# moble/scri

Hardware: AMD Instinct MI355X
Metric: timesteps/sec for full BMS transform, l_max=16, 1e5 steps; fp64 (higher is better)
Workload: dtype f64

## Files before the change

scri_amd/csrc/engine_abd.hip:

```cpp
#include "engine.h"

static int transform_abd_impl(bms_ctx* c, const double* u, const void* raw, int mem, int64_t n_times, int ell_max,
                              const bms_transformation* tr, const bms_shard* sh, double* u_out, void* raw_out, int64_t* n_times_out,
                              int64_t* first_index_out);

extern "C" int bms_transform_abd_shard(bms_ctx* c, const double* u, const void* raw, int mem, int64_t n_times, int ell_max,
                                       const bms_transformation* tr, const bms_shard* sh, double* u_out, void* raw_out,
                                       int64_t* n_times_out, int64_t* first_index_out) try {
  if (!c) return BMS_ERR_INVALID;
  return with_smaller_chunks(c, [&] { return transform_abd_impl(c, u, raw, mem, n_times, ell_max, tr, sh, u_out, raw_out, n_times_out, first_index_out); });
} BMS_CATCH(c)

static int transform_abd_impl(bms_ctx* c, const double* u, const void* raw, int mem, int64_t n_times, int ell_max,
                              const bms_transformation* tr, const bms_shard* sh, double* u_out, void* raw_out, int64_t* n_times_out,
                              int64_t* first_index_out) {
  if (!u || !raw || !tr || !u_out || !raw_out || !n_times_out) return fail(c, BMS_ERR_INVALID, "NULL argument");
  if (!valid_mem(mem)) return fail(c, BMS_ERR_INVALID, "mem is BMS_HOST or BMS_DEVICE, got %d", mem);
  HIP_TRY(c, hipSetDevice(c->device));
  const int64_t n = n_times;
  int64_t t_lo, t_hi;
  time_window(n, sh, t_lo, t_hi);
  bool regular_mesh = true;
  int rc;
  begin_setup_reuse(c);
  KnotTables kt;
  if ((rc = knot_tables_ahead(c, u, n, sh, t_lo, t_hi, kt))) return rc;
  if (kt.axis_known) {
    rc = validate_transformation(c, n, u, tr, 2);
    regular_mesh = c->tcache.regular;
  } else
    rc = validate_common(c, n, u, tr, t_lo, t_hi, &regular_mesh, 2);
  if (rc) return rc;
  const bool short_series = n < 4;
  if (short_series && sh && !(sh->data_row0 == 0 && sh->data_rows == n && sh->col_parts <= 1))
    return fail(c, BMS_ERR_UNSUPPORTED, "a series of %lld samples cannot be sharded", (long long)n);
  if ((rc = refuse_sharded_graded_axis(c, regular_mesh, sh, n))) return rc;
  if (ell_max < 0 || tr->ell_max_out < 0) return fail(c, BMS_ERR_INVALID, "bad ell_max");
  if (ell_max > MAX_ELL) return fail(c, BMS_ERR_UNSUPPORTED, "ell_max = %d is beyond %d", ell_max, MAX_ELL);
  static const int spins[6] = {2, 1, 0, -1, -2, 2};
  const int nm = (ell_max + 1) * (ell_max + 1);
  const int n_out = (tr->ell_max_out + 1) * (tr->ell_max_out + 1);
  const int lst = tr->ell_max_supertranslation;
  const cplx* st = (const cplx*)tr->supertranslation;

  hipStream_t S = c->stream;
  std::vector<cplx> c1((size_t)(lst + 1) * (lst + 1)), c2((size_t)(lst + 1) * (lst + 1));
  for (int l = 0; l <= lst; ++l)
    for (int m = -l; m <= l; ++m) {
      const cplx a = st[LM_index(l, m, 0)];
      const double f1 = std::sqrt((double)l * (l + 1.0)) / std::sqrt(2.0);
      const double f2 = 0.5 * (std::sqrt((double)l * (l + 1.0)) * (l >= 1 ? std::sqrt((l - 1.0) * (l + 2.0)) : 0.0));
      c1[LM_index(l, m, 0)] = {f1 * a.re, f1 * a.im};
      c2[LM_index(l, m, 0)] = {f2 * a.re, f2 * a.im};
    }
  const double* v = tr->boost_velocity;
  const cplx cv[4] = {{0, 0},
                      {v[0] * std::sqrt(2 * M_PI / 3), v[1] * std::sqrt(2 * M_PI / 3)},
                      {v[2] * std::sqrt(4 * M_PI / 3), 0},
                      {-v[0] * std::sqrt(2 * M_PI / 3), v[1] * std::sqrt(2 * M_PI / 3)}};
  SynthesisPlan syn5[5];
  const bool no_boost = v[0] == 0 && v[1] == 0 && v[2] == 0;
  std::vector<double> ring_theta;
  bool sep = !(sh && sh->col_parts > 1) && tr->n_theta >= 3 && !c->opt.on(OPT_NO_SEPARABLE_SYNTHESIS) &&
             (no_boost || (axis_boost_pays(c, (ell_max + 1) * (ell_max + 1), tr->n_theta, tr->n_phi) &&
                           large_synthesis_route(c, tr->n_theta, tr->n_phi, 0, ell_max) && separable_rotor_grid(c, tr, ring_theta)));
  for (int si = 0; si < 5 && sep; ++si) {
    if ((rc = build_synthesis(c, tr->n_theta, tr->n_phi, si - 2, 0, ell_max, syn5[si], no_boost ? nullptr : &ring_theta))) return rc;
    sep = syn5[si].large;
  }
  PixelTables T;
  DevPixel DP;
  PieceTables* shared = c->async_pieces ? static_cast<PieceTables*>(c->piece_tables) : nullptr;
  if (shared && c->piece_tables_valid) {
    T = shared->T;
    DP = shared->DP;
  } else {
    if ((rc = device_pixel_tables(c, tr, T, 2, 0, 0, &c1, &c2, cv, DP, sep ? 0 : column_plan(c, tr, n_out), nullptr, nullptr, nullptr, reuse_tag(sh)))) return rc;
    if (shared) {
      shared->T = T;
      shared->DP = DP;
      c->piece_tables_valid = true;
    }
  }
  const int n_cols = T.n_pix;
  const bool col_split = sh && sh->col_parts > 1;
  int cA, cB;
  if ((rc = column_range(c, sh, n_cols, cA, cB))) return rc;
  const int n_pix = cB - cA;
  int64_t i_lo, i_hi;
  if (!cached_window(c, true, i_lo, i_hi)) {
    output_window_abd(T, u, n, i_lo, i_hi);
    keep_window(c, true, i_lo, i_hi);
  }
  int64_t row0 = 0, rows_avail = n, fs_out = n;
  if (sh) {
    row0 = sh->data_row0;
    rows_avail = sh->data_rows;
    if (row0 < 0 || rows_avail < 0 || row0 + rows_avail > n || sh->out_i1 < sh->out_i0) return fail(c, BMS_ERR_INVALID, "bad shard description");
    i_lo = std::max(i_lo, sh->out_i0);
    i_hi = std::max(i_lo, std::min(i_hi, sh->out_i1));
    fs_out = sh->out_i1 - sh->out_i0;
  }
  const int64_t n_new = i_hi - i_lo;
  *n_times_out = n_new;
  if (first_index_out) *first_index_out = i_lo;
  for (int64_t i = 0; i < n_new; ++i) u_out[i] = (u[i_lo + i] - T.tt) / T.gamma;
  if (n_new == 0) return BMS_OK;
  double *d_rot = DP.rotors, *d_skewa = DP.skew_a + cA, *d_skewb = DP.skew_b + cA, *d_alpha = DP.alpha + cA, *d_ethk = DP.ethk + 2 * cA,
         *d_etha = DP.etha + 2 * cA, *d_ethetha = DP.ethetha + 2 * cA, *d_ik = DP.ik + cA, *d_ik3 = DP.ik3 + cA;
  const bool bsg = n >= 8 && regular_mesh && !c->opt.on(OPT_NO_BSPLINE);
  if (short_series) {
    void* vp;
    if ((rc = upload(c, "times", u, 8 * (size_t)n, &vp))) return rc;
    kt.d_x = (double*)vp;
  } else if ((rc = knot_tables_of_call(c, u, n, t_lo, t_hi, row0, rows_avail, bsg, shared, kt)))
    return rc;

  const long long P2 = 2LL * n_pix, ldg = round_up(P2, 16), ldb = round_up(2LL * n_cols, 128);
  const int K = 2 * nm;
  const long long brows = round_up(K, 16);
  double *d_B[5], *d_At[5] = {nullptr, nullptr, nullptr, nullptr, nullptr};
  long long ld_at = 0;
  AnalysisPlan ana[5];
  const bool sigma_eval = !sep && bsg && !short_series && rows_avail >= 8 && !c->opt.on(OPT_NO_ABD_SIGMA_EVAL);
  PixelCache& pc = c->pcache;
  const bool keep_B = !sep && pc.in_use && sizeof(double) * (size_t)brows * ldb <= SETUP_CACHE_MAX_BYTES;
  const bool have_B = keep_B && pc.B5_valid && pc.B5_ell_max == ell_max && pc.B5_cols == n_cols && pc.B5_sigma == sigma_eval;
  if (keep_B && !have_B) pc.B5_valid = false;
  for (int si = 0; si < 5; ++si) {
    char nm1[32], tag[16];
    snprintf(nm1, sizeof nm1, keep_B ? "pc_abd_B%d" : "abd_B%d", si);
    snprintf(tag, sizeof tag, "abd%d", si);
    if (!sep && have_B) {
      d_B[si] = pc.d_B5[si];
    } else if (!sep) {
      if ((rc = dev_buf_t(c, nm1, (size_t)brows * ldb, &d_B[si]))) return rc;
      HIP_TRY(c, hipMemsetAsync(d_B[si], 0, sizeof(double) * brows * ldb, S));
      TIMED(c, BMS_TAG_SETUP, launch_swsh_matrix_complex(S, d_rot, n_cols, si - 2, 0, ell_max, d_B[si], ldb));
    }
    if ((rc = build_analysis(c, tag, T.n_theta, T.n_phi, si - 2, 0, tr->ell_max_out, ana[si]))) return rc;
    if (col_split && n_pix > 0) {
      snprintf(nm1, sizeof nm1, "abd_At%d", si);
      if ((rc = part_analysis_matrix(c, ana[si], nm1, n_cols, DP.col_of_pixel, &d_At[si], &ld_at))) return rc;
    }
  }

  const long long ldG = (!col_split && analysis_reads_contiguous_rows(ana[2])) ? P2 : ldg;
  const double* d_raw;
  if ((rc = stage_in(c, "in_data", raw, mem, (size_t)6 * rows_avail * nm * 16, &d_raw))) return rc;
  double* d_out = (double*)raw_out;
  if (mem == BMS_HOST)
    if ((rc = dev_buf_t(c, "out_data", (size_t)6 * fs_out * n_out * 2, &d_out))) return rc;
  const bool fused_mix = sep && no_boost && bsg && !short_series && !c->opt.on(OPT_NO_FUSED_ABD_MIX) && large_synthesis_route(c, tr->n_theta, tr->n_phi, 0, ell_max) &&
                         abd_mix6_supported(tr->n_theta, tr->n_phi, ell_max);
  const long long ld_af = round_up(2LL * (nm + 1), 16);
  double* d_Af = nullptr;
  if (fused_mix) {
    if ((rc = dev_buf_t(c, "abd_Af", (size_t)6 * rows_avail * ld_af, &d_Af))) return rc;
    for (int f = 0; f < 6; ++f)
      TIMED(c, BMS_TAG_SPLINE_FORWARD, launch_bspline_forward_modes(S, d_raw + (size_t)f * rows_avail * nm * 2, 2LL * nm, nm, d_Af + (size_t)f * rows_avail * ld_af,
                                                                    ld_af, row0, rows_avail, n, kt.d_bsfwd, SPLINE_TILE, SPLINE_HALO, 1));
    if ((rc = rotate_into_grid_frame(c, tr, d_Af, 6 * rows_avail, ld_af / 2, 0, ell_max))) return rc;
  } else if (sep) {
    if ((rc = rotated_input_in_grid_frame(c, tr, "abd_rot_in", mem, &d_raw, 6 * rows_avail, nm, 0, ell_max))) return rc;
  }

  if (n_pix == 0) {
    for (int f = 0; f < 6; ++f) {
      if (mem == BMS_HOST)
        std::memset((char*)raw_out + (size_t)f * fs_out * n_out * 16, 0, (size_t)n_new * n_out * 16);
      else
        HIP_TRY(c, hipMemsetAsync(d_out + (size_t)f * fs_out * n_out * 2, 0, (size_t)n_new * n_out * 16, S));
    }
    HIP_TRY(c, hipStreamSynchronize(S));
    return BMS_OK;
  }

  double* d_As = nullptr;
  if (sigma_eval) {
    if ((rc = dev_buf_t(c, "abd_As", (size_t)rows_avail * ld_af, &d_As))) return rc;
    TIMED(c, BMS_TAG_SPLINE_FORWARD, launch_bspline_solve_modes(S, d_raw + (size_t)5 * rows_avail * nm * 2, 2LL * nm, nm, d_As, ld_af, row0, rows_avail,
                                                                kt.d_bsfwd, kt.d_bstab, 1));
    if (brows < (long long)nm + 1 + 8) return fail(c, BMS_ERR_HIP, "internal: the spin-2 matrix has %lld rows, sigma's offset row needs %d", brows, nm + 9);
    if (!have_B) TIMED(c, BMS_TAG_SETUP, launch_negated_row(S, DP.ethetha, d_B[4] + (size_t)nm * ldb, 2 * n_cols));
  }
  if (keep_B && !have_B) {
    pc.B5_valid = true, pc.B5_sigma = sigma_eval, pc.B5_ell_max = ell_max, pc.B5_cols = n_cols;
    for (int si = 0; si < 5; ++si) pc.d_B5[si] = d_B[si];
  }

  BsplineSpread spread = skew_spread(T, cA, cB, u);
  spread.launches = c->bwd_launches;
  const double bytes_per_row = 19.0 * ldg * 8.0;
  ChunkPlan plan;
  if ((rc = plan_chunks(c, c->ws_limit, bytes_per_row, n_new, regular_mesh, n, "six ", n_cols, plan))) return rc;
  for (int64_t c0 = i_lo; c0 < i_hi; c0 += plan.chunk) {
    const int64_t c1_ = std::min<int64_t>(c0 + plan.chunk, i_hi);
    int64_t g0, g1;
    if ((rc = chunk_rows(c, T, u, n, regular_mesh, c0, c1_, row0, rows_avail, g0, g1))) return rc;
    const int64_t rows_in = g1 - g0, rows_out = c1_ - c0;
    double *d_Y = nullptr, *d_R, *d_G;
    if (!fused_mix)
      if ((rc = dev_buf_t(c, "Y", (size_t)6 * rows_in * ldg, &d_Y))) return rc;
    if ((rc = dev_buf_t(c, "R", (size_t)6 * rows_in * ldg, &d_R))) return rc;
    if ((rc = dev_buf_t(c, "G", (size_t)6 * rows_out * ldG, &d_G))) return rc;
    AbdGrids grids;
    if (fused_mix) {
      const size_t f_stride = (size_t)rows_in * (2 * ell_max + 1) * large_analysis_jp(T.n_theta) * 2;
      double* d_F6;
      if ((rc = dev_buf_t(c, "Fsyn6", 6 * f_stride, &d_F6))) return rc;
      const double* F6[6];
      double* out6[6];
      for (int f = 0; f < 6; ++f) {
        F6[f] = d_F6 + f * f_stride;
        out6[f] = d_R + (size_t)f * rows_in * ldg;
        TIMED(c, BMS_TAG_GEMM_SYNTHESIS, launch_theta_synthesis(S, d_Af + ((size_t)f * rows_avail + (g0 - row0)) * ld_af, ld_af, rows_in, T.n_theta, 0, ell_max,
                                                                syn5[spins[f] + 2].d_T, d_F6 + f * f_stride));
      }
      TIMED(c, BMS_TAG_GEMM_SYNTHESIS, launch_phi_synthesis_mix6(S, F6, rows_in, T.n_theta, T.n_phi, ell_max, d_etha, d_ethetha,
                                                                 d_Af + (size_t)(g0 - row0) * ld_af + 2LL * nm, ld_af, out6, ldg));
    }
    for (int f = 0; f < 6 && !fused_mix; ++f) {
      grids.y[f] = d_Y + (size_t)f * rows_in * ldg;
      if (f == 5 && sigma_eval) continue;
      if (sep) {
        if ((rc = run_synthesis(c, syn5[spins[f] + 2], d_raw + ((size_t)f * rows_avail + (g0 - row0)) * nm * 2, 2LL * nm, rows_in, nullptr, grids.y[f], ldg)))
          return rc;
      } else
      {
        const int skip = spins[f] * spins[f] < nm ? spins[f] * spins[f] : 0;
        TIMED(c, BMS_TAG_GEMM_SYNTHESIS,
              launch_zgemm3m(S, d_raw + ((size_t)f * rows_avail + (g0 - row0)) * nm * 2 + 2 * skip, 2LL * nm, d_B[spins[f] + 2] + 2 * cA + (size_t)skip * ldb, ldb,
                             grids.y[f], ldg, rows_in, n_pix, K / 2 - skip, nullptr, nullptr));
      }
    }
    if (fused_mix) {
    } else if (bsg) {
      AbdGrids elim;
      for (int f = 0; f < 6; ++f) elim.y[f] = d_R + (size_t)f * rows_in * ldg;
      TIMED(c, BMS_TAG_SPLINE_FORWARD, launch_abd_mix_forward(S, grids, elim, ldg, n_pix, g0, rows_in, kt.d_bsfwd, SPLINE_TILE, SPLINE_HALO, d_alpha, d_ethk,
                                                              d_etha, d_ethetha, d_ik, d_ik3, sigma_eval ? 5 : 6));
    } else {
      TIMED(c, BMS_TAG_POINTWISE,
            launch_abd_mix(S, grids, ldg, n_pix, rows_in, kt.d_x + g0, d_alpha, d_ethk, d_etha, d_ethetha, d_ik, d_ik3));
    }
    for (int f = 0; f < 6; ++f) {
      double* Rf = d_R + (size_t)f * rows_in * ldg;
      double* Gf = d_G + (size_t)f * rows_out * ldG;
      if (short_series) {
        TIMED(c, BMS_TAG_SPLINE_BACKWARD, launch_short_series_eval(S, grids.y[f], ldg, n_pix, (int)n, kt.d_x, kt.d_x, d_skewa, d_skewb, T.tt, c0, c1_, Gf, ldG));
      } else if (f == 5 && sigma_eval) {
        SplineEval ev;
        ev.skew_a = d_skewa, ev.skew_b = d_skewb;
        if ((rc = spline_eval_args(c, kt, T, cA, cB, u, n, g0, g1, c0, c1_, Gf, ldG, ldg, ev))) return rc;
        const int skip = 4 < nm ? 4 : 0;
        TIMED(c, BMS_TAG_GEMM_SYNTHESIS, launch_zgemm3m_eval(S, d_As + (g0 - row0) * ld_af + 2 * skip, ld_af, d_B[4] + 2 * cA + (size_t)skip * ldb, ldb, rows_in,
                                                             n_pix, nm - skip + 1, DP.col_scale + 2 * cA, ev));
      } else if (bsg) {
        TIMED(c, BMS_TAG_SPLINE_BACKWARD, launch_bspline_backward_eval(S, Rf, ldg, n_pix, g0, rows_in, n, kt.d_x, kt.d_bstab, SPLINE_TILE, SPLINE_HALO,
                                                                       kt.d_x, d_skewa, d_skewb, T.tt, c0, c1_, Gf, ldG, &spread));
      } else {
        TIMED(c, BMS_TAG_SPLINE_FORWARD,
              launch_spline_forward(S, grids.y[f], Rf, ldg, n_pix, g0, rows_in, n, kt.d_x, kt.d_tab, plan.spline_tile, SPLINE_HALO));
        TIMED(c, BMS_TAG_SPLINE_BACKWARD,
              launch_spline_backward_eval(S, grids.y[f], Rf, ldg, n_pix, g0, rows_in, n, kt.d_x, kt.d_tab, plan.spline_tile, SPLINE_HALO,
                                          kt.d_x, d_skewa, d_skewb, T.tt, c0, c1_, Gf, ldG));
      }
      double* out_f = d_out + ((size_t)f * fs_out + (c0 - i_lo)) * n_out * 2;
      if (col_split) {
        TIMED(c, BMS_TAG_GEMM_ANALYSIS, launch_zgemm3m(S, Gf, ldG, d_At[spins[f] + 2] + (size_t)cA * ld_at, ld_at, out_f, 2LL * n_out, rows_out, n_out, n_pix,
                                                       nullptr, nullptr));
      } else if ((rc = run_analysis(c, ana[spins[f] + 2], Gf, rows_out, out_f, 2LL * n_out, DP.col_of_pixel, ldG)))
        return rc;
    }
  }
  if (mem == BMS_HOST) {
    for (int f = 0; f < 6; ++f)
      HIP_TRY(c, hipMemcpyAsync((char*)raw_out + (size_t)f * fs_out * n_out * 16, d_out + (size_t)f * fs_out * n_out * 2,
                                (size_t)n_new * n_out * 16, hipMemcpyDeviceToHost, S));
  }
  time_axis_commit(c, kt.times_ahead, regular_mesh);
  if (!c->async_pieces) HIP_TRY(c, hipStreamSynchronize(S));
  return BMS_OK;
}

extern "C" int bms_transform_abd_pipelined(bms_ctx* c, const double* u, const void* raw, int64_t n, int ell_max,
                                           const bms_transformation* tr, int pieces, double* u_out, void* raw_out, int64_t* n_times_out) try {
  return bms_transform_abd_pipelined_part(c, u, raw, n, ell_max, tr, pieces, 0, pieces < 1 ? 1 : pieces, u_out, raw_out, n_times_out);
} BMS_CATCH(c)

extern "C" int bms_transform_abd_pipelined_part(bms_ctx* c, const double* u, const void* raw, int64_t n, int ell_max, const bms_transformation* tr,
                                                int pieces, int piece0, int piece1, double* u_out, void* raw_out, int64_t* n_times_out) try {
  if (!c) return BMS_ERR_INVALID;
  if (!u || !raw || !tr || !u_out || !raw_out || !n_times_out) return fail(c, BMS_ERR_INVALID, "NULL argument");
  HIP_TRY(c, hipSetDevice(c->device));
  bool regular = true;
  int rc = validate_common(c, n, u, tr, 0, n, &regular);
  if (rc) return rc;
  if (!regular) return fail(c, BMS_ERR_UNSUPPORTED, "the time steps vary by more than 1e3 within 48 samples: not sharded");
  if (ell_max < 0 || tr->ell_max_out < 0) return fail(c, BMS_ERR_INVALID, "bad ell_max");
  if (ell_max > MAX_ELL) return fail(c, BMS_ERR_UNSUPPORTED, "ell_max = %d is beyond %d", ell_max, MAX_ELL);
  PixelTables T;
  int64_t i_lo, i_hi;
  if ((rc = tables_and_window(c, tr, u, n, true, T, i_lo, i_hi))) return rc;
  *n_times_out = i_hi - i_lo;
  PiecePlan P;
  plan_pieces(T, u, n, i_lo, i_hi, pieces, piece0, piece1, P);
  if (P.p1 <= P.p0) return BMS_OK;
  const int64_t n_new = i_hi - i_lo;
  const int64_t nm = (int64_t)(ell_max + 1) * (ell_max + 1), n_out = (int64_t)(tr->ell_max_out + 1) * (tr->ell_max_out + 1);
  double *d_in[2], *d_out[2];
  if ((rc = dev_buf_t(c, "pipe_in0", (size_t)6 * P.max_rows * nm * 2, &d_in[0]))) return rc;
  if ((rc = dev_buf_t(c, "pipe_in1", (size_t)6 * P.max_rows * nm * 2, &d_in[1]))) return rc;
  if ((rc = dev_buf_t(c, "pipe_out0", (size_t)6 * P.max_out * n_out * 2, &d_out[0]))) return rc;
  if ((rc = dev_buf_t(c, "pipe_out1", (size_t)6 * P.max_out * n_out * 2, &d_out[1]))) return rc;
  SharedPieceTables shared(c);
  return run_host_pipeline(
      c, P.p0, P.p1, false, true, "pipelined upload", "pipelined transfer",
      [&](int k, int slot) {
        const int64_t rows = P.r1[k] - P.r0[k];
        hipError_t e = hipSuccess;
        for (int f = 0; f < 6 && e == hipSuccess; ++f)
          e = hipMemcpyAsync(d_in[slot] + (size_t)f * rows * nm * 2, (const char*)raw + ((size_t)f * n + P.r0[k]) * nm * 16, (size_t)rows * nm * 16,
                             hipMemcpyHostToDevice, c->pipe_up);
        return e;
      },
      [&](int k, int slot) {
        const bms_shard sh = P.shard(k);
        int64_t got = 0, first = 0;
        const int rc2 = transform_abd_impl(c, u, d_in[slot], BMS_DEVICE, n, ell_max, tr, &sh, u_out + (P.cut[k] - i_lo), d_out[slot], &got, &first);
        return rc2 ? rc2 : piece_produced(c, P, k, got, first);
      },
// ... 22 lines not shown
```

scri_amd/csrc/env.h:

```cpp
#pragma once
#include <cstdlib>
#include <cstring>

namespace bms {

#define BMS_ROUTE_OPTIONS(X)                                   \
  X(TRACE, "TRACE")                                            \
  X(ROTATE_VALU, "ROTATE_VALU")                                \
  X(ROTATE_STAGED, "ROTATE_STAGED")                            \
  X(NO_FUSED_ANALYSIS, "NO_FUSED_ANALYSIS")                    \
  X(NO_LARGE_ANALYSIS, "NO_LARGE_ANALYSIS")                    \
  X(NO_SPLIT_ANALYSIS, "NO_SPLIT_ANALYSIS")                    \
  X(NO_PLAN_CACHE, "NO_PLAN_CACHE")                            \
  X(AXIS_BOOST_MIN_WORK, "AXIS_BOOST_MIN_WORK")                \
  X(NO_AXIS_BOOST_SEPARABLE, "NO_AXIS_BOOST_SEPARABLE")        \
  X(NO_SPLIT_SYNTHESIS, "NO_SPLIT_SYNTHESIS")                  \
  X(NO_COLUMN_SORT, "NO_COLUMN_SORT")                          \
  X(NO_BSPLINE, "NO_BSPLINE")                                  \
  X(WALK_FIRST, "WALK_FIRST")                                  \
  X(NO_SMALL_DENSE, "NO_SMALL_DENSE")                          \
  X(NO_SEPARABLE_SYNTHESIS, "NO_SEPARABLE_SYNTHESIS")          \
  X(NO_LARGE_SYNTHESIS, "NO_LARGE_SYNTHESIS")                  \
  X(NO_GEMM_EVAL, "NO_GEMM_EVAL")                              \
  X(SYNTHESIS_EVAL, "SYNTHESIS_EVAL")                          \
  X(NO_SYNTHESIS_EVAL, "NO_SYNTHESIS_EVAL")                    \
  X(TWO_SWEEPS, "TWO_SWEEPS")                                  \
  X(GEMM_EVAL_STEP, "GEMM_EVAL_STEP")                          \
  X(GRID_MULTIPLY_FULL_GRID, "GRID_MULTIPLY_FULL_GRID")        \
  X(NO_ABD_SIGMA_EVAL, "NO_ABD_SIGMA_EVAL")                    \
  X(NO_FUSED_ABD_MIX, "NO_FUSED_ABD_MIX")                      \
  X(NO_ROTATE_PIPELINE, "NO_ROTATE_PIPELINE")

enum RouteOpt : int {
#define X(e, n) OPT_##e,
  BMS_ROUTE_OPTIONS(X)
#undef X
      OPT_COUNT,
  OPT_ASYNC_RETURN = OPT_COUNT,
  OPT_TOTAL
};

inline const char* route_option_name(int i) {
  static const char* const names[OPT_TOTAL] = {
#define X(e, n) n,
      BMS_ROUTE_OPTIONS(X)
#undef X
      "ASYNC_RETURN",
  };
  return (i >= 0 && i < OPT_TOTAL) ? names[i] : nullptr;
}

inline int route_option_index(const char* name) {
  if (!name) return -1;
  if (std::strncmp(name, "SCRI_AMD_", 9) == 0) name += 9;
  for (int i = 0; i < OPT_TOTAL; ++i)
    if (std::strcmp(name, route_option_name(i)) == 0) return i;
  return -1;
}

struct RouteOptions {
  long long v[OPT_TOTAL] = {0};
  RouteOptions() {
    v[OPT_AXIS_BOOST_MIN_WORK] = -1;
    v[OPT_ASYNC_RETURN] = 1;
  }
  bool on(RouteOpt o) const { return v[o] != 0; }
  void read_environment() {
    for (int i = 0; i < OPT_TOTAL; ++i) {
      char full[64] = "SCRI_AMD_";
      std::strncat(full, i == OPT_ASYNC_RETURN ? "NO_ASYNC_RETURN" : route_option_name(i), sizeof full - 10);
      const char* e = std::getenv(full);
      if (!e) continue;
      if (i == OPT_AXIS_BOOST_MIN_WORK) {
        v[i] = std::atoll(e) > 0 ? std::atoll(e) : 0;
      } else if (i == OPT_GEMM_EVAL_STEP) {
        v[i] = std::atoll(e);
      } else if (i == OPT_ASYNC_RETURN) {
        v[i] = (e[0] == 0 || std::strcmp(e, "0") == 0) ? 1 : 0;
      } else {
        v[i] = (e[0] == 0 || std::strcmp(e, "0") == 0) ? 0 : 1;
      }
    }
  }
};

}

#ifdef SCRI_AMD_PROBES
#define BMS_PROBE_ENV(name) std::getenv(name)
#define BMS_PROBES 1
#else
#define BMS_PROBE_ENV(name) (static_cast<const char*>(nullptr))
#define BMS_PROBES 0
#endif
```

scri_amd/csrc/kernels.h:

```cpp
#pragma once
#include <algorithm>
#include <vector>
#include <hip/hip_runtime.h>
#include <stdint.h>

#include "env.h"

#include <map>
#include <mutex>
#include <utility>

namespace bms {

constexpr long long GRID_Y_MAX = 65535;

inline int lds_per_workgroup(int dev) {
  int lds = 0, v = 0;
  if (hipDeviceGetAttribute(&v, hipDeviceAttributeSharedMemPerBlockOptin, dev) == hipSuccess) lds = std::max(lds, v);
  if (hipDeviceGetAttribute(&v, hipDeviceAttributeMaxSharedMemoryPerBlock, dev) == hipSuccess) lds = std::max(lds, v);
  (void)hipGetLastError();
  if (lds <= 64 * 1024) lds = 160 * 1024;
  return lds;
}

// ... 40 lines not shown
void rotate_resident_pack(const RotResPlan& P, int ell, const double* Delta, double* image);
hipError_t launch_rotate_modes_resident(hipStream_t stream, double* data, long long n_times, long long ld, const double* RaRb,
                                        long long rotor_stride, const double* tab_global, const RotResPlan& P, size_t lds_bytes,
                                        unsigned int* counter, int n_cu);

struct ModeMapSide {
  const double* data;
  long long ld;
  const int* idx;
  const double* coef;
  int conj;
};
hipError_t launch_row_norm(hipStream_t stream, const double* data, long long ld, long long n_rows, int n_cols, int take_sqrt, double* out);
hipError_t launch_series_to_blocks(hipStream_t stream, const double* in, long long ld_in, double* out, long long n_rows, int n_modes, int F);
hipError_t launch_blocks_to_series(hipStream_t stream, const double* in, long long block_rows, double* out, long long n_rows, int n_cols, int F);
hipError_t launch_mode_map(hipStream_t stream, double* out, long long ld_out, long long n_rows, int n_cols, const ModeMapSide& A,
                           const ModeMapSide& B, const double* row_scale);

hipError_t launch_swsh_matrix(hipStream_t stream, const double* rotors , int n_pix, int spin,
                              int ell_min, int ell_max, double* Bmat, long long ldb);
hipError_t launch_swsh_matrix_complex(hipStream_t stream, const double* rotors, int n_pix, int spin, int ell_min,
                                      int ell_max, double* Bmat, long long ldb);
hipError_t launch_quadrature_matrix(hipStream_t stream, const double* rotors, const double* w_pix, int n_pix, int spin,
                                    int ell_min, int ell_max, double* Wmat, long long ldw);
hipError_t launch_swsh_values(hipStream_t stream, const double* rotors, int n_pix, int spin, int ell_min, int ell_max,
                              double* Y );

struct PixelSpec;
struct PixelOut;
hipError_t launch_pixel_tables(hipStream_t stream, const PixelSpec& P, const PixelOut& O, int n_pix, const int* perm);
int pixel_sort_max();
hipError_t launch_pixel_sort(hipStream_t stream, const PixelSpec& P, int n_theta, int n_phi, int by_key, int* perm, int* inv);

hipError_t launch_dft_matrix(hipStream_t stream, int n_phi, int L, double* B, long long ldb);
hipError_t launch_theta_table(hipStream_t stream, const double* Y, const double* w_theta, int n_theta, int n_out, double* T);
hipError_t launch_theta_quadrature(hipStream_t stream, const double* F, long long n_rows, int n_theta, int nm, int n_out,
                                   const int* m_index, const double* T, double* out, long long ldo);
constexpr int MAX_THETA_SEPARABLE = 104;
int large_analysis_supported(int n_theta, int n_phi, int L);
int large_analysis_jp(int n_theta);
hipError_t launch_analysis_large(hipStream_t stream, const double* G, long long ldg, long long n_rows, int n_theta, int n_phi,
                                 int L, int ell_min_out, const double* T, double* F, double* out, long long ldo);
struct FusedGeom;
int fused_analysis_supported(int n_theta, int n_phi, int L, int n_out);
size_t fused_dft_table_size(int n_phi, int L);
hipError_t launch_dft_cs_matrix(hipStream_t stream, int n_phi, int L, double* D);
hipError_t launch_analysis_fused(hipStream_t stream, const double* G, long long ldg, long long n_rows, int n_theta, int n_phi,
                                 int L, int n_out, const int* m_index, const double* T, const double* D, double* out,
                                 long long ldo, const int* col_of_pixel, int spin, bool allow_split = true);

hipError_t launch_short_series_eval(hipStream_t stream, const double* Y, long long ld, int n_cols, int n, const double* x,
                                    const double* base, const double* skew_a, const double* skew_b, double tt, long long i_lo,
                                    long long i_hi, double* out, long long ldo);

struct SynGeom {
  int n_theta, n_phi, L, n_modes, nk;
  int nth, nph;
  int n_lists, len;
};
int synthesis_split_plan(int n_theta, int n_phi, int ell_min, int ell_max, SynGeom& g, std::vector<int>& meta, size_t& lds_bytes,
                         int& nt, int& len);
size_t synthesis_split_scale_bytes(int n_theta, int n_phi);
hipError_t launch_synthesis_split(hipStream_t stream, const double* A, long long lda, long long n_rows, const SynGeom& g, int nt,
                                  const double* Tsyn, const int* meta, const double* off, double* Y, long long ldy, size_t lds_bytes,
                                  int n_cu, const double* scale = nullptr);

struct SplineEval;
int synthesis_eval_supported(const SynGeom& g, int nt, size_t* lds_bytes, int* nph, int* ring_rows, int* staged_abscissae);
hipError_t launch_synthesis_eval(hipStream_t stream, const double* A, long long lda, long long n_rows, const SynGeom& g, int nt,
                                 const double* Tsyn, const int* meta, const SplineEval& e, double s_min, double s_max, int n_cu);
hipError_t launch_sub_const_modes(hipStream_t stream, double* Y, long long ld, long long n_rows, int n, const int* col, const double* c, int one_col);

int large_synthesis_supported(int n_theta, int n_phi, int ell_min, int ell_max);
hipError_t launch_synthesis_large(hipStream_t stream, const double* A, long long lda, long long n_rows, int n_theta, int n_phi,
                                  int ell_min, int ell_max, const double* Tsyn, const double* off, double* F, double* Y,
                                  long long ldy, const double* scale = nullptr);

hipError_t launch_theta_synthesis(hipStream_t stream, const double* A, long long lda, long long n_rows, int n_theta, int ell_min,
                                  int ell_max, const double* Tsyn, double* F);
int abd_mix6_supported(int n_theta, int n_phi, int ell_max);
hipError_t launch_phi_synthesis_mix6(hipStream_t stream, const double* const F6[6], long long n_rows, int n_theta, int n_phi,
                                     int ell_max, const double* eth_alpha, const double* etheth_alpha, const double* cst, long long ldc,
                                     double* const out6[6], long long ldo);

hipError_t launch_dgemm(hipStream_t stream, const double* A, long long lda, const double* B, long long ldb, double* C,
                        long long ldc, long long M, int N, int K, const double* col_off, const double* col_scale);

hipError_t launch_zgemm3m(hipStream_t stream, const double* A, long long lda, const double* B, long long ldb, double* C,
                          long long ldc, long long M, int N, int K, const double* col_off, const double* col_scale);

struct BsplineTable;
struct SplineEval {
  const BsplineTable* table;
  const double* x;
  const double* skew_a;
  const double* skew_b;
  double tt;
  long long g0;
  long long n_knots;
  long long i_lo, i_hi;
  double* out;
  long long ldo;
  int search_halfwidth;
  double inv_dx;
  unsigned long long* stats;
  double* side;
  long long side_ld;
  int step = 0;
};
long long zgemm3m_eval_side_rows(long long M);
hipError_t launch_zgemm3m_eval(hipStream_t stream, const double* A, long long lda, const double* B, long long ldb, long long M, int N,
                               int K, const double* col_scale, const SplineEval& e);

struct SplineTable {
  double P, Q, A, C;
};
hipError_t launch_spline_table(hipStream_t stream, const double* x, long long n, SplineTable* table, long long j0,
                               long long j1);
hipError_t launch_spline_forward(hipStream_t stream, const double* Y, double* R, long long ld, int n_cols ,
                                 long long g0, long long n_rows, long long n_knots, const double* x,
                                 const SplineTable* table, int tile, int halo);
hipError_t launch_spline_backward_eval(hipStream_t stream, const double* Y, const double* R, long long ld, int n_cols,
                                       long long g0, long long n_rows, long long n_knots, const double* x,
                                       const SplineTable* table, int tile, int halo, const double* base,
                                       const double* skew_a, const double* skew_b, double tt, long long i_lo,
                                       long long i_hi, double* out, long long ldo);

struct BsplineTable {
  double m[16];
  double G, D;
  double x;
  double pad;
};
struct BsplineForward {
  double P, A, E, x;
};
hipError_t launch_bspline_table(hipStream_t stream, const double* x, long long n, BsplineTable* table, BsplineForward* fwd,
                                long long j_lo , long long j0, long long j1);
hipError_t launch_bspline_forward_modes(hipStream_t stream, const double* A, long long lda, int n_modes, double* Aout,
                                        long long ldo, long long g0, long long n_rows, long long n_knots,
                                        const BsplineForward* table, int tile, int halo, int with_ones);
hipError_t launch_bspline_backward_modes(hipStream_t stream, const double* A, long long lda, int n_cols, double* Aout, long long ldo,
                                         long long g0, long long n_rows, const BsplineTable* table, int tile, int halo);
hipError_t launch_bspline_solve_modes(hipStream_t stream, const double* A, long long lda, int n_modes, double* Aout, long long ldo,
                                      long long g0, long long n_rows, const BsplineForward* fwd, const BsplineTable* table, int with_ones);
struct AbdGrids;
hipError_t launch_abd_mix_forward(hipStream_t stream, const AbdGrids& Y, const AbdGrids& R, long long ld, int n_cols, long long g0,
                                  long long n_rows, const BsplineForward* table, int tile, int halo, const double* alpha,
                                  const double* ethk_over_k, const double* eth_alpha, const double* etheth_alpha,
                                  const double* inv_k, const double* inv_k3, int n_fields = 6 );
hipError_t launch_negated_row(hipStream_t stream, const double* off, double* row, int n);
struct BsplineSpread {
  double skew_rate_range, skew_offset_range;
  const double* x;
  unsigned long long* launches = nullptr;
};
hipError_t launch_bspline_backward_eval(hipStream_t stream, const double* C, long long ld, int n_cols, long long g0,
                                        long long n_rows, long long n_knots, const double* x, const BsplineTable* table,
                                        int tile, int halo, const double* base, const double* skew_a, const double* skew_b,
                                        double tt, long long i_lo, long long i_hi, double* out, long long ldo, const BsplineSpread* spread = nullptr);

hipError_t launch_spline_slopes(hipStream_t stream, const double* R, double* S, long long ld, int n_cols, long long n,
                                const SplineTable* table, int tile, int halo);
long long spline_prefix_carry_size(long long n, int n_cols);
hipError_t launch_spline_prefix_levels(hipStream_t stream, const double* Y, const double* S, long long ld, int n_cols, long long n,
                                       const double* x, double* Pall, long long level_stride, double* carry, int levels);
// ... 141 lines not shown
```

scri_amd/csrc/kernels_synthesis_large.hip:

```cpp
#include <hip/hip_runtime.h>

#include <cstdlib>
#include <type_traits>

#include "kernels.h"
#include "wigner.h"

namespace bms {

typedef double v4d_t __attribute__((ext_vector_type(4)));

template <int KL, int NTJ>
__global__ __launch_bounds__(256, NTJ <= 4 ? 3 : 2) void theta_synthesis_mfma_kernel(const double* __restrict__ A, long long lda, long long n_rows,
                                                                   int n_theta, int L, int ell_min, int jp, int rows_per_block,
                                                                   const double* __restrict__ Tsyn, double* __restrict__ F) {
  constexpr int PQ = 4 * KL + 2;
  __shared__ double As[4][16 * PQ];
  const int wave = threadIdx.x >> 6, lane = threadIdx.x & 63, fi = lane & 15, fk = lane >> 4;
  const int mi = blockIdx.x, m = mi - L, nm = 2 * L + 1;
  const int tile0 = blockIdx.z * NTJ;
  const int am = m < 0 ? -m : m;
  const int l0 = am > ell_min ? am : ell_min;
  const int nl = L - l0 + 1;
  const int ks = (nl + 3) / 4;
// ... 240 lines not shown
    const auto [t, rt, rings] = phi_item<4>(item, mt, n_theta);
    const long long pix0 = (long long)(4 * rt) * n_phi;
    const int n_el = rings * n_phi;
#pragma unroll
    for (int it = 0; it < MAXIT; ++it) {
      const int e = lane + 64 * it;
      const long long p = pix0 + (e < n_el ? e : 0);
      tB[it] = *reinterpret_cast<const double2*>(a.eth_alpha + 2 * p);
      tE[it] = *reinterpret_cast<const double2*>(a.etheth_alpha + 2 * p);
    }
#pragma unroll
    for (int pass = 0; pass < 3; ++pass) {
      double2* Ft = sm + (size_t)(2 * pass) * tile;
#pragma unroll
      for (int i = 0; i < NPRE; ++i) {
        const int e = lane + 64 * i;
        if (e < 8 * nm) Ft[e] = pre[i];
      }
      if (pass == 0) M6_LOAD(item, 1)
      if (pass == 1) M6_LOAD(item, 2)
      if (pass == 2 && item + gridDim.x < n_items) M6_LOAD(item + gridDim.x, 0)
      v4d_t u[NTC], v[NTC];
      phi_folded_products<4>(Ft, ab * 4 * nm, ag, part, fk, L, km, bc, bs, u, v);
      const double2 f0a = Ft[L * 4 + fk], f0b = Ft[4 * nm + L * 4 + fk];
      __builtin_amdgcn_s_waitcnt(0xc07f);
      double2* Ga = sm + (size_t)(2 * pass) * tile + fk * n_phi;
      double2* Gb = Ga + tile;
#pragma unroll
      for (int n = 0; n < NTC; ++n) {
        const int k = 16 * n + fi;
        if (k < nk) {
          const double uax = f0a.x + u[n][0], uay = f0a.y + u[n][1], ubx = f0b.x + u[n][2], uby = f0b.y + u[n][3];
          Ga[k] = double2{uax + v[n][0], uay + v[n][1]};
          Gb[k] = double2{ubx + v[n][2], uby + v[n][3]};
          const int k2 = n_phi - k;
          if (k >= 1 && k2 != k) {
            Ga[k2] = double2{uax - v[n][0], uay - v[n][1]};
            Gb[k2] = double2{ubx - v[n][2], uby - v[n][3]};
          }
        }
      }
    }
    const double cv = a.cst[t * a.ldc];
#pragma unroll
    for (int it = 0; it < MAXIT; ++it) {
      const int e = lane + 64 * it;
      if (e < n_el) {
        const long long p = pix0 + e;
        cplx f[6];
#pragma unroll
        for (int i = 0; i < 6; ++i) {
          const double2 w = sm[(size_t)i * tile + e];
          f[i] = {w.x, w.y};
        }
        const double2 EE = tE[it];
        const cplx X = {-tB[it].x, -tB[it].y};
        auto axpy = [](cplx tt, cplx X, double c, cplx ff) {
          cplx r = cmul(tt, X);
          return cplx{r.re + c * ff.re, r.im + c * ff.im};
        };
        cplx t0 = f[4];
        t0 = axpy(t0, X, -4.0, f[3]);
        t0 = axpy(t0, X, 6.0, f[2]);
        t0 = axpy(t0, X, -4.0, f[1]);
        t0 = axpy(t0, X, 1.0, f[0]);
        cplx t1 = {-f[4].re, -f[4].im};
        t1 = axpy(t1, X, 3.0, f[3]);
        t1 = axpy(t1, X, -3.0, f[2]);
        t1 = axpy(t1, X, 1.0, f[1]);
        cplx t2 = f[4];
        t2 = axpy(t2, X, -2.0, f[3]);
        t2 = axpy(t2, X, 1.0, f[2]);
        cplx t3 = {-f[4].re, -f[4].im};
        t3 = axpy(t3, X, 1.0, f[3]);
        const cplx mixed[6] = {t0, t1, t2, t3, f[4], {f[5].re - EE.x * cv, f[5].im - EE.y * cv}};
#pragma unroll
        for (int i = 0; i < 6; ++i) *reinterpret_cast<double2*>(a.out[i] + t * a.ldo + 2 * p) = double2{mixed[i].re, mixed[i].im};
      }
    }
  }
#undef M6_LOAD
}

int large_synthesis_supported(int n_theta, int n_phi, int ell_min, int ell_max) {
  const int nk = n_phi / 2 + 1;
  return n_theta >= 2 && n_theta <= 104 && n_phi >= 1 && nk <= 64 && ell_max >= 1 && ell_max <= 33 && ell_min >= 0 && ell_min <= ell_max;
}

template <int N, class Go>
static hipError_t with_k_steps(int k, Go go) {
  using std::integral_constant;
  if (k <= 5) return go(integral_constant<int, 5>{}, integral_constant<int, N>{});
  if (k <= 7) return go(integral_constant<int, 7>{}, integral_constant<int, N>{});
  return go(integral_constant<int, 9>{}, integral_constant<int, N>{});
}

template <class Go>
static hipError_t with_phi_instance(int n_phi, int L, Go go) {
  const int km = (L + 3) / 4, ntc = (n_phi / 2 + 1 + 15) / 16;
  if (ntc <= 2) return with_k_steps<2>(km, go);
  if (ntc == 3) return with_k_steps<3>(km, go);
  return with_k_steps<4>(km, go);
}

hipError_t launch_theta_synthesis(hipStream_t stream, const double* A, long long lda, long long n_rows, int n_theta, int ell_min,
                                  int ell_max, const double* Tsyn, double* F) {
  if (n_rows <= 0) return hipSuccess;
  const int L = ell_max, nm = 2 * L + 1, jp = large_analysis_jp(n_theta);
  static const int rows_per_block = BMS_PROBE_ENV("SCRI_AMD_TS_ROWS") ? atoi(BMS_PROBE_ENV("SCRI_AMD_TS_ROWS")) : 256;
  const int kl = (L + 1 - ell_min + 3) / 4, ntj_all = (n_theta + 15) / 16;
  static const int ts_split = BMS_PROBE_ENV("SCRI_AMD_TS_SPLIT") ? atoi(BMS_PROBE_ENV("SCRI_AMD_TS_SPLIT")) : 0;
  const int parts = ts_split && ntj_all > 4 ? 2 : 1;
  const int ntj = (ntj_all + parts - 1) / parts;
  const dim3 grid(nm, (unsigned)((n_rows + rows_per_block - 1) / rows_per_block), parts);
  auto go = [&](auto KL, auto NTJ) {
    hipLaunchKernelGGL((theta_synthesis_mfma_kernel<KL.value, NTJ.value>), grid, dim3(256), 0, stream, A, lda, n_rows, n_theta, L, ell_min,
                       jp, rows_per_block, Tsyn, F);
    return hipGetLastError();
  };
  if (ntj <= 3) return with_k_steps<3>(kl, go);
  if (ntj == 4) return with_k_steps<4>(kl, go);
  if (ntj <= 5) return with_k_steps<5>(kl, go);
  return with_k_steps<7>(kl, go);
}

hipError_t launch_synthesis_large(hipStream_t stream, const double* A, long long lda, long long n_rows, int n_theta, int n_phi,
                                  int ell_min, int ell_max, const double* Tsyn, const double* off, double* F, double* Y,
                                  long long ldy, const double* scale) {
  if (n_rows <= 0) return hipSuccess;
  hipError_t e = launch_theta_synthesis(stream, A, lda, n_rows, n_theta, ell_min, ell_max, Tsyn, F);
  if (e != hipSuccess) return e;
  const int L = ell_max, nm = 2 * L + 1, jp = large_analysis_jp(n_theta);
  const int n_modes = (L + 1) * (L + 1) - ell_min * ell_min;
  const size_t lds = sizeof(double2) * ((size_t)nm * 8 + (size_t)8 * n_phi);
  const long long items = n_rows * ((n_theta + 7) / 8);
  const unsigned grid = (unsigned)(items < 256 * 8 ? items : 256 * 8);
  return with_phi_instance(n_phi, L, [&](auto KM, auto NTC) {
    hipLaunchKernelGGL((phi_synthesis_folded_kernel<KM.value, NTC.value>), dim3(grid), dim3(64), lds, stream, F, n_rows, n_theta, n_phi, L,
                       jp, off, A + 2LL * n_modes, lda, scale, Y, ldy);
    return hipGetLastError();
  });
}

int abd_mix6_supported(int n_theta, int n_phi, int ell_max) {
  return large_synthesis_supported(n_theta, n_phi, 0, ell_max) && 2 * ell_max + 1 <= n_phi && (size_t)6 * 4 * n_phi * 16 <= 53 * 1024;
}

hipError_t launch_phi_synthesis_mix6(hipStream_t stream, const double* const F6[6], long long n_rows, int n_theta, int n_phi,
                                     int ell_max, const double* eth_alpha, const double* etheth_alpha, const double* cst, long long ldc,
                                     double* const out6[6], long long ldo) {
  if (n_rows <= 0) return hipSuccess;
  Mix6Args a;
  for (int f = 0; f < 6; ++f) a.F[f] = F6[f], a.out[f] = out6[f];
  a.eth_alpha = eth_alpha, a.etheth_alpha = etheth_alpha, a.cst = cst, a.ldc = ldc, a.ldo = ldo;
  const int L = ell_max, jp = large_analysis_jp(n_theta);
  const size_t lds = sizeof(double2) * (size_t)6 * 4 * n_phi;
  const long long items = n_rows * ((n_theta + 3) / 4);
  const unsigned grid = (unsigned)(items < 256 * 4 ? items : 256 * 4);
  return with_phi_instance(n_phi, L, [&](auto KM, auto NTC) {
    hipError_t e = allow_dynamic_lds((const void*)phi_synthesis_mix6_kernel<KM.value, NTC.value>);
    if (e != hipSuccess) return e;
    hipLaunchKernelGGL((phi_synthesis_mix6_kernel<KM.value, NTC.value>), dim3(grid), dim3(64), lds, stream, a, n_rows, n_theta, n_phi, L, jp);
    return hipGetLastError();
  });
}

}
```

Before: 21.90 million.

## Fuse ABD phi synthesis and mixing with B-spline evaluation in one kernel

```diff
diff --git a/scri_amd/csrc/engine_abd.hip b/scri_amd/csrc/engine_abd.hip
--- a/scri_amd/csrc/engine_abd.hip
+++ b/scri_amd/csrc/engine_abd.hip
@@ -1,4 +1,6 @@
 #include "engine.h"
+
+constexpr int ABD_PHI_EVAL_MIN_ELL = 8;
 
 static int transform_abd_impl(bms_ctx* c, const double* u, const void* raw, int mem, int64_t n_times, int ell_max,
                               const bms_transformation* tr, const bms_shard* sh, double* u_out, void* raw_out, int64_t* n_times_out,
@@ -153,13 +155,20 @@
     if ((rc = dev_buf_t(c, "out_data", (size_t)6 * fs_out * n_out * 2, &d_out))) return rc;
   const bool fused_mix = sep && no_boost && bsg && !short_series && !c->opt.on(OPT_NO_FUSED_ABD_MIX) && large_synthesis_route(c, tr->n_theta, tr->n_phi, 0, ell_max) &&
                          abd_mix6_supported(tr->n_theta, tr->n_phi, ell_max);
+  const bool want_phi_eval = c->opt.on(OPT_ABD_PHI_EVAL) || (!c->opt.on(OPT_NO_ABD_PHI_EVAL) && ell_max >= ABD_PHI_EVAL_MIN_ELL);
+  const bool phi_eval = fused_mix && want_phi_eval && rows_avail >= 8;
   const long long ld_af = round_up(2LL * (nm + 1), 16);
   double* d_Af = nullptr;
   if (fused_mix) {
     if ((rc = dev_buf_t(c, "abd_Af", (size_t)6 * rows_avail * ld_af, &d_Af))) return rc;
-    for (int f = 0; f < 6; ++f)
-      TIMED(c, BMS_TAG_SPLINE_FORWARD, launch_bspline_forward_modes(S, d_raw + (size_t)f * rows_avail * nm * 2, 2LL * nm, nm, d_Af + (size_t)f * rows_avail * ld_af,
-                                                                    ld_af, row0, rows_avail, n, kt.d_bsfwd, SPLINE_TILE, SPLINE_HALO, 1));
+    for (int f = 0; f < 6; ++f) {
+      const double* in_f = d_raw + (size_t)f * rows_avail * nm * 2;
+      double* af = d_Af + (size_t)f * rows_avail * ld_af;
+      if (phi_eval)
+        TIMED(c, BMS_TAG_SPLINE_FORWARD, launch_bspline_solve_modes(S, in_f, 2LL * nm, nm, af, ld_af, row0, rows_avail, kt.d_bsfwd, kt.d_bstab, 1));
+      else
+        TIMED(c, BMS_TAG_SPLINE_FORWARD, launch_bspline_forward_modes(S, in_f, 2LL * nm, nm, af, ld_af, row0, rows_avail, n, kt.d_bsfwd, SPLINE_TILE, SPLINE_HALO, 1));
+    }
     if ((rc = rotate_into_grid_frame(c, tr, d_Af, 6 * rows_avail, ld_af / 2, 0, ell_max))) return rc;
   } else if (sep) {
     if ((rc = rotated_input_in_grid_frame(c, tr, "abd_rot_in", mem, &d_raw, 6 * rows_avail, nm, 0, ell_max))) return rc;
@@ -199,10 +208,11 @@
     int64_t g0, g1;
     if ((rc = chunk_rows(c, T, u, n, regular_mesh, c0, c1_, row0, rows_avail, g0, g1))) return rc;
     const int64_t rows_in = g1 - g0, rows_out = c1_ - c0;
-    double *d_Y = nullptr, *d_R, *d_G;
+    double *d_Y = nullptr, *d_R = nullptr, *d_G;
     if (!fused_mix)
       if ((rc = dev_buf_t(c, "Y", (size_t)6 * rows_in * ldg, &d_Y))) return rc;
-    if ((rc = dev_buf_t(c, "R", (size_t)6 * rows_in * ldg, &d_R))) return rc;
+    if (!phi_eval)
+      if ((rc = dev_buf_t(c, "R", (size_t)6 * rows_in * ldg, &d_R))) return rc;
     if ((rc = dev_buf_t(c, "G", (size_t)6 * rows_out * ldG, &d_G))) return rc;
     AbdGrids grids;
     if (fused_mix) {
@@ -217,8 +227,17 @@
         TIMED(c, BMS_TAG_GEMM_SYNTHESIS, launch_theta_synthesis(S, d_Af + ((size_t)f * rows_avail + (g0 - row0)) * ld_af, ld_af, rows_in, T.n_theta, 0, ell_max,
                                                                 syn5[spins[f] + 2].d_T, d_F6 + f * f_stride));
       }
-      TIMED(c, BMS_TAG_GEMM_SYNTHESIS, launch_phi_synthesis_mix6(S, F6, rows_in, T.n_theta, T.n_phi, ell_max, d_etha, d_ethetha,
-                                                                 d_Af + (size_t)(g0 - row0) * ld_af + 2LL * nm, ld_af, out6, ldg));
+      if (phi_eval) {
+        if (rows_in < 4) return fail(c, BMS_ERR_HIP, "internal: a chunk of %lld coefficient rows holds no window", (long long)rows_in);
+        SplineEval ev;
+        ev.table = kt.d_bstab, ev.x = kt.d_x, ev.skew_a = nullptr, ev.skew_b = d_skewb, ev.tt = T.tt, ev.g0 = g0, ev.n_knots = n;
+        ev.i_lo = c0, ev.i_hi = c1_, ev.out = d_G, ev.ldo = ldG;
+        ev.search_halfwidth = 0, ev.inv_dx = 0.0, ev.side = nullptr, ev.side_ld = 0, ev.stats = nullptr;
+        TIMED(c, BMS_TAG_GEMM_SYNTHESIS, launch_phi_synthesis_mix6_eval(S, d_F6, (long long)f_stride, rows_in, T.n_theta, T.n_phi, ell_max, d_etha, d_ethetha,
+                                                                        d_Af + (size_t)(g0 - row0) * ld_af + 2LL * nm, ld_af, ev, (long long)rows_out * ldG));
+      } else
+        TIMED(c, BMS_TAG_GEMM_SYNTHESIS, launch_phi_synthesis_mix6(S, F6, rows_in, T.n_theta, T.n_phi, ell_max, d_etha, d_ethetha,
+                                                                   d_Af + (size_t)(g0 - row0) * ld_af + 2LL * nm, ld_af, out6, ldg));
     }
     for (int f = 0; f < 6 && !fused_mix; ++f) {
       grids.y[f] = d_Y + (size_t)f * rows_in * ldg;
@@ -247,7 +266,8 @@
     for (int f = 0; f < 6; ++f) {
       double* Rf = d_R + (size_t)f * rows_in * ldg;
       double* Gf = d_G + (size_t)f * rows_out * ldG;
-      if (short_series) {
+      if (phi_eval) {
+      } else if (short_series) {
         TIMED(c, BMS_TAG_SPLINE_BACKWARD, launch_short_series_eval(S, grids.y[f], ldg, n_pix, (int)n, kt.d_x, kt.d_x, d_skewa, d_skewb, T.tt, c0, c1_, Gf, ldG));
       } else if (f == 5 && sigma_eval) {
         SplineEval ev;
diff --git a/scri_amd/csrc/env.h b/scri_amd/csrc/env.h
--- a/scri_amd/csrc/env.h
+++ b/scri_amd/csrc/env.h
@@ -37,6 +37,8 @@
 #undef X
       OPT_COUNT,
   OPT_ASYNC_RETURN = OPT_COUNT,
+  OPT_ABD_PHI_EVAL,
+  OPT_NO_ABD_PHI_EVAL,
   OPT_TOTAL
 };
 
@@ -46,6 +48,8 @@
       BMS_ROUTE_OPTIONS(X)
 #undef X
       "ASYNC_RETURN",
+      "ABD_PHI_EVAL",
+      "NO_ABD_PHI_EVAL",
   };
   return (i >= 0 && i < OPT_TOTAL) ? names[i] : nullptr;
 }
diff --git a/scri_amd/csrc/kernels.h b/scri_amd/csrc/kernels.h
--- a/scri_amd/csrc/kernels.h
+++ b/scri_amd/csrc/kernels.h
@@ -146,6 +146,10 @@
 hipError_t launch_phi_synthesis_mix6(hipStream_t stream, const double* const F6[6], long long n_rows, int n_theta, int n_phi,
                                      int ell_max, const double* eth_alpha, const double* etheth_alpha, const double* cst, long long ldc,
                                      double* const out6[6], long long ldo);
+constexpr int ABD_EVAL_BLOCK = 128;
+hipError_t launch_phi_synthesis_mix6_eval(hipStream_t stream, const double* F, long long f_stride, long long n_rows, int n_theta, int n_phi,
+                                          int ell_max, const double* eth_alpha, const double* etheth_alpha, const double* cst, long long ldc,
+                                          const SplineEval& e, long long out_stride);
 
 hipError_t launch_dgemm(hipStream_t stream, const double* A, long long lda, const double* B, long long ldb, double* C,
                         long long ldc, long long M, int N, int K, const double* col_off, const double* col_scale);
diff --git a/scri_amd/csrc/kernels_synthesis_large.hip b/scri_amd/csrc/kernels_synthesis_large.hip
--- a/scri_amd/csrc/kernels_synthesis_large.hip
+++ b/scri_amd/csrc/kernels_synthesis_large.hip
@@ -346,6 +346,219 @@
 #undef M6_LOAD
 }
 
+struct Mix6EvalArgs {
+  long long f_stride;
+  long long n_rows;
+  long long g0, n;
+  long long i_lo, i_hi;
+  long long ldo, out_stride;
+  long long ldc;
+  int n_theta, n_phi, L, jp, block;
+};
+constexpr int M6E_XW = 512;
+
+template <int KM, int NC>
+__global__ __launch_bounds__(128 * NC) void phi_synthesis_mix6_eval_kernel(const double* __restrict__ F, const double* __restrict__ eth_alpha,
+                                                                          const double* __restrict__ etheth_alpha, const double* __restrict__ cst,
+                                                                          const double* __restrict__ skew_b, const double* __restrict__ xg,
+                                                                          const BsplineTable* __restrict__ tabg, double* __restrict__ out,
+                                                                          Mix6EvalArgs a) {
+  extern __shared__ __attribute__((aligned(16))) double2 sm[];
+  constexpr int NT = 128 * NC;
+  const int L = a.L, nm = 2 * L + 1, n_phi = a.n_phi, jp = a.jp;
+  const int fsz = 24 * nm;
+  double* xw = reinterpret_cast<double*>(sm + 2 * fsz);
+  int* first_row = reinterpret_cast<int*>(xw + M6E_XW);
+  const int tid = threadIdx.x, wave = __builtin_amdgcn_readfirstlane(tid >> 6), lane = tid & 63, fi = lane & 15, fk = lane >> 4;
+  const int nk = n_phi / 2 + 1, mt = (a.n_theta + 3) / 4;
+  const long long tb = blockIdx.x / mt;
+  const int rt = (int)(blockIdx.x - tb * mt);
+  const int rings = a.n_theta - 4 * rt < 4 ? a.n_theta - 4 * rt : 4;
+  const long long fA = a.g0, fB = a.g0 + a.n_rows - 3;
+  const long long f0 = fA + tb * a.block;
+  const long long f1 = f0 + a.block < fB ? f0 + a.block : fB;
+  const int n_blk_rows = (int)(f1 - f0) + 3;
+  const long long row0 = f0 - fA;
+
+  const int k = 16 * (wave >> 1) + fi;
+  const int side = wave & 1;
+  double bc[KM][1], bs[KM][1];
+#pragma unroll
+  for (int s = 0; s < KM; ++s) {
+    const int m = 4 * s + fk + 1;
+    double sn = 0.0, co = 0.0;
+    if (k < nk && m <= L) sincospi(2.0 * (double)(((long long)m * k) % n_phi) / (double)n_phi, &sn, &co);
+    bc[s][0] = co, bs[s][0] = sn;
+  }
+  const int km = (L + 3) / 4;
+  const int ab = fi >> 3, ag = fi & 3, part = (fi >> 2) & 1;
+
+  const bool ok = k < nk && fk < rings && (side == 0 || (k >= 1 && 2 * k != n_phi));
+  const long long pix = ok ? (long long)(4 * rt + fk) * n_phi + (side ? n_phi - k : k) : 0;
+  const double2 tB = *reinterpret_cast<const double2*>(eth_alpha + 2 * pix), tE = *reinterpret_cast<const double2*>(etheth_alpha + 2 * pix);
+  const double sb = skew_b[pix];
+  const double vs = side ? -1.0 : 1.0;
+
+  const int n_i = (int)(a.i_hi - a.i_lo);
+  const double* __restrict__ bp = xg + a.i_lo;
+  const double inf = __builtin_huge_val();
+  const double blk_lo = f0 == fA ? -inf : xg[f0 + 1];
+  int ic;
+  {
+    int lo = 0, hi = f0 == fA ? 0 : n_i;
+    while (lo < hi) {
+      const int mid = (lo + hi) >> 1;
+      if (bp[mid] + sb < blk_lo)
+        lo = mid + 1;
+      else
+        hi = mid;
+    }
+    ic = ok ? lo : n_i;
+  }
+  if (tid == 0) *first_row = n_i;
+  __syncthreads();
+  if (ic < n_i) atomicMin(first_row, ic);
+  __syncthreads();
+  const int i_a = *first_row;
+  for (int e = tid; e < M6E_XW; e += NT) {
+    const int i = i_a + e;
+    xw[e] = bp[i < n_i ? i : (n_i > 0 ? n_i - 1 : 0)];
+  }
+  typedef const double __attribute__((address_space(3))) * lds_cdp;
+  const lds_cdp xwl = (lds_cdp)xw;
+  auto xs = [&](int i) -> double {
+    double x = inf;
+    if (i < n_i) {
+      if (i - i_a < M6E_XW)
+        x = xwl[i - i_a];
+      else
+        x = bp[i];
+    }
+    return x;
+  };
+
+  constexpr int NPRE = (24 * (8 * KM + 1) + NT - 1) / NT;
+  long long goff[NPRE];
+#pragma unroll
+  for (int i = 0; i < NPRE; ++i) {
+    const int e = tid + NT * i;
+    const int q = e >> 2, r = e & 3;
+    const int fld = q / nm, mi = q - fld * nm;
+    goff[i] = (e < fsz && r < rings) ? fld * a.f_stride + ((long long)mi * jp + 4 * rt + r) * 2 : -1;
+  }
+  const long long f_row = (long long)nm * jp * 2;
+  double2 pre[NPRE];
+  double cvn = 0.0;
+#define M6E_LOAD(S)                                                                                                   \
+  {                                                                                                                   \
+    const double* f_ = F + (row0 + (S)) * f_row;                                                                      \
+    _Pragma("unroll") for (int i = 0; i < NPRE; ++i)                                                                  \
+        pre[i] = goff[i] >= 0 ? *reinterpret_cast<const double2*>(f_ + goff[i]) : double2{0.0, 0.0};                   \
+    cvn = cst[(row0 + (S)) * a.ldc];                                                                                  \
+  }
+  double W[4][12];
+#pragma unroll
+  for (int r = 0; r < 4; ++r)
+#pragma unroll
+    for (int e = 0; e < 12; ++e) W[r][e] = 0.0;
+  double xcur = 0.0;
+  M6E_LOAD(0)
+
+  for (int s = 0; s <= n_blk_rows; ++s) {
+    {
+      {
+        const bool produce = s < n_blk_rows;
+        double2* Ft = sm + (s & 1) * fsz;
+        const double cv = cvn;
+        if (produce) {
+#pragma unroll
+          for (int i = 0; i < NPRE; ++i) {
+            const int e = tid + NT * i;
+            if (e < fsz) Ft[e] = pre[i];
+          }
+        }
+        __syncthreads();
+        if (s == 0) xcur = xs(ic);
+        if (s >= 4) {
+          const long long f = f0 + s - 4, jj = f + 1;
+          const double xlo = xg[jj];
+          const double xhi = (f == a.n - 4 || f == fB - 1) ? inf : xg[jj + 1];
+          const double* __restrict__ tm = tabg[jj].m;
+          const double m00 = tm[0], m01 = tm[1], m02 = tm[2], m03 = tm[3], m10 = tm[4], m11 = tm[5], m12 = tm[6], m13 = tm[7];
+          const double m20 = tm[8], m21 = tm[9], m22 = tm[10], m23 = tm[11], m30 = tm[12], m31 = tm[13], m32 = tm[14], m33 = tm[15];
+          const double(&q0)[12] = W[0], (&q1)[12] = W[1], (&q2)[12] = W[2], (&q3)[12] = W[3];
+          {
+            int c = ic;
+            double xc = xcur;
+            while (c < n_i && xc + sb < xhi) {
+              const double t = (xc - xlo) + sb;
+              const double b0 = fma(fma(fma(m30, t, m20), t, m10), t, m00);
+              const double b1 = fma(fma(fma(m31, t, m21), t, m11), t, m01);
+              const double b2 = fma(fma(fma(m32, t, m22), t, m12), t, m02);
+              const double b3 = fma(fma(fma(m33, t, m23), t, m13), t, m03);
+              double* o = out + (long long)c * a.ldo + 2 * pix;
+#pragma unroll
+              for (int fl = 0; fl < 6; ++fl) {
+                const int e = 2 * fl;
+                double2 v;
+                v.x = fma(b3, q3[e], fma(b2, q2[e], fma(b1, q1[e], b0 * q0[e])));
+                v.y = fma(b3, q3[e + 1], fma(b2, q2[e + 1], fma(b1, q1[e + 1], b0 * q0[e + 1])));
+                *reinterpret_cast<double2*>(o + fl * a.out_stride) = v;
+              }
+              ++c;
+              xc = xs(c);
+            }
+            ic = c, xcur = xc;
+          }
+        }
+        if (s + 1 < n_blk_rows) M6E_LOAD(s + 1)
+        if (produce) {
+          double raw[12];
+#pragma unroll
+          for (int pass = 0; pass < 3; ++pass) {
+            v4d_t u[1], v[1];
+            phi_folded_products<4>(Ft, (2 * pass + ab) * 4 * nm, ag, part, fk, L, km, bc, bs, u, v);
+            const double2 f0a = Ft[(2 * pass) * 4 * nm + L * 4 + fk], f0b = Ft[(2 * pass + 1) * 4 * nm + L * 4 + fk];
+            const double uax = f0a.x + u[0][0], uay = f0a.y + u[0][1], ubx = f0b.x + u[0][2], uby = f0b.y + u[0][3];
+            raw[4 * pass + 0] = fma(vs, v[0][0], uax), raw[4 * pass + 1] = fma(vs, v[0][1], uay);
+            raw[4 * pass + 2] = fma(vs, v[0][2], ubx), raw[4 * pass + 3] = fma(vs, v[0][3], uby);
+          }
+          {
+            cplx f[6];
+#pragma unroll
+            for (int i = 0; i < 6; ++i) f[i] = {raw[2 * i], raw[2 * i + 1]};
+            const cplx X = {-tB.x, -tB.y};
+            auto axpy = [](cplx tt, cplx X, double c, cplx ff) {
+              cplx rr = cmul(tt, X);
+              return cplx{rr.re + c * ff.re, rr.im + c * ff.im};
+            };
+            cplx t0 = f[4];
+            t0 = axpy(t0, X, -4.0, f[3]);
+            t0 = axpy(t0, X, 6.0, f[2]);
+            t0 = axpy(t0, X, -4.0, f[1]);
+            t0 = axpy(t0, X, 1.0, f[0]);
+            cplx t1 = {-f[4].re, -f[4].im};
+            t1 = axpy(t1, X, 3.0, f[3]);
+            t1 = axpy(t1, X, -3.0, f[2]);
+            t1 = axpy(t1, X, 1.0, f[1]);
+            cplx t2 = f[4];
+            t2 = axpy(t2, X, -2.0, f[3]);
+            t2 = axpy(t2, X, 1.0, f[2]);
+            cplx t3 = {-f[4].re, -f[4].im};
+            t3 = axpy(t3, X, 1.0, f[3]);
+            const cplx mixed[6] = {t0, t1, t2, t3, f[4], {f[5].re - tE.x * cv, f[5].im - tE.y * cv}};
+#pragma unroll
+            for (int e = 0; e < 12; ++e) W[0][e] = W[1][e], W[1][e] = W[2][e], W[2][e] = W[3][e];
+#pragma unroll
+            for (int i = 0; i < 6; ++i) W[3][2 * i] = mixed[i].re, W[3][2 * i + 1] = mixed[i].im;
+          }
+        }
+      }
+    }
+  }
+#undef M6E_LOAD
+}
+
 int large_synthesis_supported(int n_theta, int n_phi, int ell_min, int ell_max) {
   const int nk = n_phi / 2 + 1;
   return n_theta >= 2 && n_theta <= 104 && n_phi >= 1 && nk <= 64 && ell_max >= 1 && ell_max <= 33 && ell_min >= 0 && ell_min <= ell_max;
@@ -429,4 +642,30 @@
   });
 }
 
-}
+hipError_t launch_phi_synthesis_mix6_eval(hipStream_t stream, const double* F, long long f_stride, long long n_rows, int n_theta, int n_phi,
+                                          int ell_max, const double* eth_alpha, const double* etheth_alpha, const double* cst, long long ldc,
+                                          const SplineEval& e, long long out_stride) {
+  if (e.i_hi <= e.i_lo) return hipSuccess;
+  if (n_rows < 4 || !abd_mix6_supported(n_theta, n_phi, ell_max) || e.i_hi - e.i_lo >= (1LL << 31)) return hipErrorInvalidValue;
+  const int L = ell_max, nm = 2 * L + 1;
+  Mix6EvalArgs a;
+  a.f_stride = f_stride, a.n_rows = n_rows, a.g0 = e.g0, a.n = e.n_knots, a.i_lo = e.i_lo, a.i_hi = e.i_hi;
+  a.ldo = e.ldo, a.out_stride = out_stride, a.ldc = ldc;
+  a.n_theta = n_theta, a.n_phi = n_phi, a.L = L, a.jp = large_analysis_jp(n_theta), a.block = ABD_EVAL_BLOCK;
+  const size_t lds = sizeof(double2) * (size_t)2 * 24 * nm + sizeof(double) * M6E_XW + 16;
+  const long long n_blocks = (n_rows - 3 + a.block - 1) / a.block;
+  const long long items = n_blocks * ((n_theta + 3) / 4);
+  if (items >= (1LL << 31)) return hipErrorInvalidValue;
+  const int km = (L + 3) / 4, ntc = (n_phi / 2 + 1 + 15) / 16;
+  auto go = [&](auto KM, auto NC) {
+    hipError_t er = allow_dynamic_lds((const void*)phi_synthesis_mix6_eval_kernel<KM.value, NC.value>);
+    if (er != hipSuccess) return er;
+    hipLaunchKernelGGL((phi_synthesis_mix6_eval_kernel<KM.value, NC.value>), dim3((unsigned)items), dim3(128 * NC.value), lds, stream, F, eth_alpha,
+                       etheth_alpha, cst, e.skew_b, e.x, e.table, e.out, a);
+    return hipGetLastError();
+  };
+  if (ntc <= 1) return with_k_steps<1>(km, go);
+  return with_k_steps<4>(km, go);
+}
+
+}
```

New measurement: 21.92 million (median of 4 runs). About the same (+0.1%).
